# tyfeld/MMaDA-Parallel

Hardware: NVIDIA H100
Metric: denoised_tokens_per_sec (higher is better)
Workload: dtype bf16; 1 GPU; MMaDA-Parallel-A 8B, 1 prompt per GPU, 512x512 (1024 VQ tokens) + 256 text tokens, timesteps=64, text_steps=128, cfg_img=4.0, cfg_scale=0, temperature=1.0, text_temperature=0 (BASELINE configs[1]); seq_len=2414, parallelism=replicas x1 (independent prompts, no collective), weights=synthetic normal(0, 0.02) bf16, seeded, l2=16.2 GB of weights streamed per forward >> 50 MB L2 (no flush needed)

## Files before the change

### mmada_parallel_b200/csrc/attention.cu

```cuda
#include "mmdp_internal.h"
#include "ptx.cuh"

#include <stdlib.h>

#include <map>
#include <mutex>
#include <utility>

namespace mmdp {

static constexpr int kAttnThreads = 384;
static constexpr int kQBytes = 128 * 128 * 2;
template <int BKV> struct AttnCfg {
    static constexpr int kKBytes = BKV * 128 * 2;
    static constexpr int kVBytes = 128 * BKV * 2;
    static constexpr int kSmem = kQBytes + 2 * (kKBytes + kVBytes) + 1024  + 256 ;
};

__device__ __forceinline__ float ex2_approx(float x) {
    float y;
    asm("ex2.approx.ftz.f32 %0, %1;" : "=f"(y) : "f"(x));
    return y;
}

struct AttnSegs {
    int n;
    int start[kMaxSegs + 1];
    int tile0[kMaxSegs + 1];
};

template <int kBKV, bool kPacked>
__device__ __forceinline__ void attention_body(const CUtensorMap& tmQ, const CUtensorMap& tmK, const CUtensorMap& tmVt,
                                               __nv_bfloat16* __restrict__ out, int H, int L, int d_model, float scale_log2,
                                               int n_full, int splits, float* __restrict__ part_ws, int Lq, const AttnSegs* segs) {
    constexpr int kKBytes = AttnCfg<kBKV>::kKBytes, kVBytes = AttnCfg<kBKV>::kVBytes;
    extern __shared__ uint8_t smem_raw[];
    uint8_t* smem = reinterpret_cast<uint8_t*>((reinterpret_cast<uintptr_t>(smem_raw) + 1023) & ~uintptr_t(1023));
    uint8_t* sQ = smem;
    uint8_t* sK = sQ + kQBytes;
    uint8_t* sV = sK + 2 * kKBytes;
    uint64_t* bars = reinterpret_cast<uint64_t*>(sV + 2 * kVBytes);
    uint64_t* q_full = bars + 0;
    uint64_t* k_full = bars + 1;
    uint64_t* k_empty = bars + 3;
    uint64_t* v_full = bars + 5;
    uint64_t* v_empty = bars + 7;

    const int warp = threadIdx.x >> 5, lane = threadIdx.x & 31, wg = warp >> 2;
    int n_qt = (Lq + 127) / 128;
    int n_kv_all = (L + kBKV - 1) / kBKV;
    int tile = blockIdx.x, piece = -1;
    if ((int)blockIdx.x >= n_full) {
        const int t = (int)blockIdx.x - n_full;
        tile = n_full + t / splits;
        piece = t - (t / splits) * splits;
// ... 38 lines not shown
        setmaxnreg_dec<40>();
        if (warp == 0 && elect_one_sync()) {
            const int qrow0 = (kPacked ? seg0 : b * Lq) + qt * 128;
            mbar_expect_tx(q_full, kQBytes);
            tma_load_2d(sQ, &tmQ, q_full, h * 128, qrow0);
            tma_load_2d(sQ + kQBytes / 2, &tmQ, q_full, h * 128 + 64, qrow0);
            for (int j = 0; j < n_kv; ++j) {
                const int st = j & 1;
                const uint32_t ph = (j >> 1) & 1;
                const int kv0 = (jb + j) * kBKV;
                mbar_wait(&k_empty[st], ph ^ 1);
                mbar_expect_tx(&k_full[st], kKBytes);
                tma_load_2d(sK + st * kKBytes, &tmK, &k_full[st], h * 128, (kPacked ? seg0 : b * L) + kv0);
                tma_load_2d(sK + st * kKBytes + kKBytes / 2, &tmK, &k_full[st], h * 128 + 64, (kPacked ? seg0 : b * L) + kv0);
                mbar_wait(&v_empty[st], ph ^ 1);
                mbar_expect_tx(&v_full[st], kVBytes);
                tma_load_2d(sV + st * kVBytes, &tmVt, &v_full[st], kv0, (b * H + h) * 128);
                if (kBKV == 128) tma_load_2d(sV + st * kVBytes + kVBytes / 2, &tmVt, &v_full[st], kv0 + 64, (b * H + h) * 128);
            }
        }
        __syncwarp();
        return;
    }

    setmaxnreg_inc<232>();
    const int half = wg - 1;
    const int r0 = half * 64 + (warp & 3) * 16 + (lane >> 2), c0 = 2 * (lane & 3);
    const uint32_t aQ = smem_u32(sQ) + half * (64 * 128);
    float o[64];
#pragma unroll
    for (int i = 0; i < 64; ++i) o[i] = 0.f;
    float m_run[2] = {-INFINITY, -INFINITY}, l_run[2] = {0.f, 0.f};
    mbar_wait(q_full, 0);
    for (int j = 0; j < n_kv; ++j) {
        const int st = j & 1;
        const uint32_t ph = (j >> 1) & 1;
        const int nvalid = L - (jb + j) * kBKV;
        float sacc[kBKV / 2];
        const uint32_t aK = smem_u32(sK + st * kKBytes);
        mbar_wait(&k_full[st], ph);
        wgmma_fence();
#pragma unroll
        for (int kk = 0; kk < 8; ++kk)
        {
            const uint64_t qd = smem_desc_kmajor_sw128(aQ + (kk >> 2) * (kQBytes / 2)) + (kk & 3) * 2;
            const uint64_t kd = smem_desc_kmajor_sw128(aK + (kk >> 2) * (kKBytes / 2)) + (kk & 3) * 2;
            if constexpr (kBKV == 128) wgmma_bf16_ss_n128(sacc, qd, kd, kk != 0);
            else wgmma_bf16_ss_n64(sacc, qd, kd, kk != 0);
        }
        wgmma_commit();
        wgmma_wait<0>();
        reg_fence(sacc);
        __syncwarp();
        if (lane == 0) mbar_arrive(&k_empty[st]);
        if (nvalid < kBKV) {
#pragma unroll
            for (int jj = 0; jj < kBKV / 8; ++jj)
#pragma unroll
                for (int e = 0; e < 2; ++e)
                    if (8 * jj + c0 + e >= nvalid) { sacc[4 * jj + e] = -INFINITY; sacc[4 * jj + 2 + e] = -INFINITY; }
        }
        float alpha[2], mneg[2];
#pragma unroll
        for (int hh = 0; hh < 2; ++hh) {
            float mx = sacc[2 * hh];
#pragma unroll
            for (int jj = 0; jj < kBKV / 8; ++jj) mx = fmaxf(mx, fmaxf(sacc[4 * jj + 2 * hh], sacc[4 * jj + 2 * hh + 1]));
            mx = fmaxf(mx, __shfl_xor_sync(0xffffffffu, mx, 1));
            mx = fmaxf(mx, __shfl_xor_sync(0xffffffffu, mx, 2));
            const float m_new = fmaxf(m_run[hh], mx);
            alpha[hh] = ex2_approx((m_run[hh] - m_new) * scale_log2);
            m_run[hh] = m_new;
            mneg[hh] = -m_new * scale_log2;
        }
        uint32_t pa[kBKV / 4];
        float rsum[2] = {0.f, 0.f};
#pragma unroll
        for (int jj = 0; jj < kBKV / 8; ++jj)
#pragma unroll
            for (int hh = 0; hh < 2; ++hh) {
                const float p0 = ex2_approx(fmaf(sacc[4 * jj + 2 * hh], scale_log2, mneg[hh]));
                const float p1 = ex2_approx(fmaf(sacc[4 * jj + 2 * hh + 1], scale_log2, mneg[hh]));
                rsum[hh] += p0 + p1;
                pa[2 * jj + hh] = pack_bf16x2(p0, p1);
            }
#pragma unroll
        for (int hh = 0; hh < 2; ++hh) l_run[hh] = fmaf(l_run[hh], alpha[hh], rsum[hh]);
#pragma unroll
        for (int jj = 0; jj < 16; ++jj) {
            o[4 * jj] *= alpha[0]; o[4 * jj + 1] *= alpha[0];
            o[4 * jj + 2] *= alpha[1]; o[4 * jj + 3] *= alpha[1];
        }
        const uint32_t aV = smem_u32(sV + st * kVBytes);
        mbar_wait(&v_full[st], ph);
        wgmma_fence();
#pragma unroll
        for (int kk = 0; kk < kBKV / 16; ++kk) {
            const uint32_t a[4] = {pa[4 * kk], pa[4 * kk + 1], pa[4 * kk + 2], pa[4 * kk + 3]};
            wgmma_bf16_rs_n128(o, a, smem_desc_kmajor_sw128(aV + (kk >> 2) * (kVBytes / 2)) + (kk & 3) * 2, 1);
        }
        wgmma_commit();
        wgmma_wait<0>();
        reg_fence(o);
        __syncwarp();
        if (lane == 0) mbar_arrive(&v_empty[st]);
    }
#pragma unroll
    for (int hh = 0; hh < 2; ++hh) {
        l_run[hh] += __shfl_xor_sync(0xffffffffu, l_run[hh], 1);
        l_run[hh] += __shfl_xor_sync(0xffffffffu, l_run[hh], 2);
    }
#pragma unroll
    for (int hh = 0; hh < 2; ++hh) {
        const int r = r0 + 8 * hh, qrow = qt * 128 + r;
        if (qrow >= Lq) continue;
        if (piece >= 0) {
            float* slot = part_ws + (size_t)((tile - n_full) * splits + piece) * (128 * 128 + 256);
            if ((lane & 3) == 0) {
                slot[128 * 128 + r] = m_run[hh];
                slot[128 * 128 + 128 + r] = l_run[hh];
            }
#pragma unroll
            for (int jj = 0; jj < 16; ++jj)
                *reinterpret_cast<float2*>(slot + (size_t)r * 128 + 8 * jj + c0) = make_float2(o[4 * jj + 2 * hh], o[4 * jj + 2 * hh + 1]);
        } else {
            const float inv_l = 1.0f / l_run[hh];
            __nv_bfloat16* orow = out + (size_t)((kPacked ? seg0 : b * Lq) + qrow) * d_model + h * 128;
#pragma unroll
            for (int jj = 0; jj < 16; ++jj)
                *reinterpret_cast<uint32_t*>(orow + 8 * jj + c0) = pack_bf16x2(o[4 * jj + 2 * hh] * inv_l, o[4 * jj + 2 * hh + 1] * inv_l);
        }
    }
}

template <int kBKV>
__global__ void __launch_bounds__(kAttnThreads, 1)
attention_kernel(const __grid_constant__ CUtensorMap tmQ, const __grid_constant__ CUtensorMap tmK,
                 const __grid_constant__ CUtensorMap tmVt, __nv_bfloat16* __restrict__ out, int H, int L, int d_model,
                 float scale_log2, int n_full, int splits, float* __restrict__ part_ws, int Lq) {
    attention_body<kBKV, false>(tmQ, tmK, tmVt, out, H, L, d_model, scale_log2, n_full, splits, part_ws, Lq, nullptr);
}

template <int kBKV>
__global__ void __launch_bounds__(kAttnThreads, 1)
attention_packed_kernel(const __grid_constant__ CUtensorMap tmQ, const __grid_constant__ CUtensorMap tmK,
                        const __grid_constant__ CUtensorMap tmVt, __nv_bfloat16* __restrict__ out, int H, int d_model,
                        float scale_log2, int n_full, int splits, float* __restrict__ part_ws, const __grid_constant__ AttnSegs segs) {
    attention_body<kBKV, true>(tmQ, tmK, tmVt, out, H, 0, d_model, scale_log2, n_full, splits, part_ws, 0, &segs);
}

template <bool kPacked>
__device__ __forceinline__ void attention_combine_body(const float* __restrict__ part_ws, __nv_bfloat16* __restrict__ out, int H,
                                                       int Lq, int d_model, float scale_log2, int n_full, int splits,
                                                       const AttnSegs* segs) {
    int n_qt = (Lq + 127) / 128;
    const int st = blockIdx.x, r = blockIdx.y, c = threadIdx.x;
    pdl_launch_dependents();
    pdl_wait();
    const int tile = n_full + st;
    int seg = 0, seg0 = 0, tl = tile;
    if constexpr (kPacked) {
        for (int i = 1; i < segs->n; ++i)
            if (tile >= segs->tile0[i]) seg = i;
        seg0 = segs->start[seg];
        Lq = segs->start[seg + 1] - seg0;
        n_qt = (Lq + 127) / 128;
        tl = tile - segs->tile0[seg];
    }
    const int qt = tl % n_qt, h = (tl / n_qt) % H, b = kPacked ? seg : tile / (n_qt * H);
    const int qrow = qt * 128 + r;
    if (qrow >= Lq) return;
    const float* base = part_ws + (size_t)st * splits * (128 * 128 + 256);
    float m = -INFINITY;
    for (int i = 0; i < splits; ++i) m = fmaxf(m, base[(size_t)i * (128 * 128 + 256) + 128 * 128 + r]);
    float o = 0.f, l = 0.f;
    for (int i = 0; i < splits; ++i) {
        const float* slot = base + (size_t)i * (128 * 128 + 256);
        const float w = exp2f((slot[128 * 128 + r] - m) * scale_log2);
        o = fmaf(w, slot[(size_t)r * 128 + c], o);
        l = fmaf(w, slot[128 * 128 + 128 + r], l);
    }
// ... 38 lines not shown
        for (int t = first; t < tiles; ++t)
            if (sp > kvb_of(t) / 2) sp = kvb_of(t) / 2;
        auto empty_piece = [&](int s) {
            for (int t = first; t < tiles; ++t) {
                const int n_kvb = kvb_of(t);
                if ((s - 1) * ((n_kvb + s - 1) / s) >= n_kvb) return true;
            }
            return false;
        };
        while (sp >= 2 && empty_piece(sp)) --sp;
        return sp;
    };
    if (split_tail && tiles > slots && (tiles % slots) > 0 && (tiles % slots) * 4 <= slots) {
        n_split = tiles % slots;
        splits = fit_splits(slots / n_split, tiles - n_split);
        if (splits >= 2) n_full = tiles - n_split; else { n_split = 0; splits = 1; }
    } else if (split_tail && tiles * 2 <= slots) {
        splits = fit_splits(slots / tiles, 0);
        if (splits >= 2) { n_split = tiles; n_full = 0; } else splits = 1;
    }
}

template <class Kernel>
static int attn_smem_attr(Kernel kernel, int smem, unsigned long long& attr_set) {
    int dev = 0;
    MMDP_CUDA(cudaGetDevice(&dev));
    if (!(attr_set >> (dev & 63) & 1ull)) {
        MMDP_CUDA(cudaFuncSetAttribute(kernel, cudaFuncAttributeMaxDynamicSharedMemorySize, smem));
        attr_set |= 1ull << (dev & 63);
    }
    return 0;
}

template <int kBKV>
static int attention_launch(const __nv_bfloat16* q, const __nv_bfloat16* k, const __nv_bfloat16* vt, __nv_bfloat16* out, int B, int H,
                            int L, int Lpad, float scale, cudaStream_t stream, int Lq) {
    constexpr int kAttnSmem = AttnCfg<kBKV>::kSmem;
    if (B <= 0 || H <= 0 || L <= 0) return set_error("attention: empty problem");
    if (Lq <= 0) Lq = L;
    if (Lpad < L || (Lpad % 8)) return set_error("attention: Lpad must be >= L and a multiple of 8");
    const int d_model = H * 128;
    CUtensorMap tmQ, tmK, tmVt;
    if (make_tmap_2d_bf16(&tmQ, q, (uint64_t)B * Lq, (uint64_t)d_model, (uint64_t)d_model, 128, 64)) return -1;
    if (make_tmap_2d_bf16(&tmK, k, (uint64_t)B * L, (uint64_t)d_model, (uint64_t)d_model, kBKV, 64)) return -1;
    if (make_tmap_2d_bf16(&tmVt, vt, (uint64_t)B * H * 128, (uint64_t)Lpad, (uint64_t)Lpad, 128, 64)) return -1;
    const int n_qt = (Lq + 127) / 128, n_kvb = (L + kBKV - 1) / kBKV;
    const int tiles = n_qt * H * B;
    int n_full, n_split, splits;
    plan_split_tail(tiles, [&](int) { return n_kvb; }, n_full, n_split, splits);
    float* part_ws = nullptr;
    if (n_split > 0 && attn_part_workspace(stream, (size_t)n_split * splits * (128 * 128 + 256) * sizeof(float), &part_ws)) return -1;
    const int grid = n_full + n_split * splits;
    const float scale_log2 = scale * 1.4426950408889634f;
    const bool pdl = pdl_mode() != 0;
    LaunchScope ls(LK_ATTN, 4.0 * B * H * (double)Lq * L * 128, stream);
    static unsigned long long attr_set = 0;
    if (attn_smem_attr(attention_kernel<kBKV>, kAttnSmem, attr_set)) return -1;
    MMDP_CUDA(launch_ex(attention_kernel<kBKV>, dim3(grid), dim3(kAttnThreads), kAttnSmem, stream, pdl, false, tmQ, tmK, tmVt, out, H, L,
                        d_model, scale_log2, n_full, splits, part_ws, Lq));
    if (n_split > 0)
        MMDP_CUDA(launch_ex(attention_combine_kernel, dim3(n_split, 128), dim3(128), 0, stream, pdl, false, (const float*)part_ws, out, H, Lq,
                            d_model, scale_log2, n_full, splits));
    return 0;
}

template <int kBKV>
static int attention_packed_launch(const __nv_bfloat16* q, const __nv_bfloat16* k, const __nv_bfloat16* vt, __nv_bfloat16* out,
                                   const SegTable& segs, int H, int Lpad, float scale, cudaStream_t stream) {
    constexpr int kAttnSmem = AttnCfg<kBKV>::kSmem;
    if (segs.n <= 0 || segs.n > kMaxSegs || H <= 0) return set_error("attention_packed: %d sequences (1 to %d)", segs.n, kMaxSegs);
    if (Lpad % 8) return set_error("attention_packed: Lpad must be a multiple of 8");
    AttnSegs as{};
    as.n = segs.n;
    double work = 0;
    for (int s = 0; s <= segs.n; ++s) {
        as.start[s] = segs.start[s];
        if (s == segs.n) break;
        const int len = segs.start[s + 1] - segs.start[s];
        if (len <= 0 || len > Lpad) return set_error("attention_packed: sequence %d has length %d (Lpad %d)", s, len, Lpad);
        as.tile0[s + 1] = as.tile0[s] + (len + 127) / 128 * H;
        work += 4.0 * H * (double)len * len * 128;
    }
    const int M = segs.start[segs.n], tiles = as.tile0[segs.n], d_model = H * 128;
    CUtensorMap tmQ, tmK, tmVt;
    if (make_tmap_2d_bf16(&tmQ, q, (uint64_t)M, (uint64_t)d_model, (uint64_t)d_model, 128, 64)) return -1;
    if (make_tmap_2d_bf16(&tmK, k, (uint64_t)M, (uint64_t)d_model, (uint64_t)d_model, kBKV, 64)) return -1;
    if (make_tmap_2d_bf16(&tmVt, vt, (uint64_t)segs.n * H * 128, (uint64_t)Lpad, (uint64_t)Lpad, 128, 64)) return -1;
    auto kvb_of = [&](int t) {
        int s = 0;
        while (s + 1 < segs.n && t >= as.tile0[s + 1]) ++s;
        return (segs.start[s + 1] - segs.start[s] + kBKV - 1) / kBKV;
    };
    int n_full, n_split, splits;
    plan_split_tail(tiles, kvb_of, n_full, n_split, splits);
    float* part_ws = nullptr;
    if (n_split > 0 && attn_part_workspace(stream, (size_t)n_split * splits * (128 * 128 + 256) * sizeof(float), &part_ws)) return -1;
    const int grid = n_full + n_split * splits;
    const float scale_log2 = scale * 1.4426950408889634f;
    const bool pdl = pdl_mode() != 0;
    LaunchScope ls(LK_ATTN, work, stream);
    static unsigned long long attr_set = 0;
    if (attn_smem_attr(attention_packed_kernel<kBKV>, kAttnSmem, attr_set)) return -1;
    MMDP_CUDA(launch_ex(attention_packed_kernel<kBKV>, dim3(grid), dim3(kAttnThreads), kAttnSmem, stream, pdl, false, tmQ, tmK, tmVt, out,
                        H, d_model, scale_log2, n_full, splits, part_ws, as));
    if (n_split > 0)
        MMDP_CUDA(launch_ex(attention_packed_combine_kernel, dim3(n_split, 128), dim3(128), 0, stream, pdl, false, (const float*)part_ws,
                            out, H, d_model, scale_log2, n_full, splits, as));
    return 0;
}

int attention_fwd(const __nv_bfloat16* q, const __nv_bfloat16* k, const __nv_bfloat16* vt, __nv_bfloat16* out, int B, int H, int L,
                  int Lpad, float scale, cudaStream_t stream, int Lq) {
    const int version = opt(OPT_ATTN_VERSION);
    if (version == 7) return attention_launch<64>(q, k, vt, out, B, H, L, Lpad, scale, stream, Lq);
    if (version != 6) return set_error("attention: unknown kernel generation %d (6 or 7)", version);
    return attention_launch<128>(q, k, vt, out, B, H, L, Lpad, scale, stream, Lq);
}

int attention_packed_fwd(const __nv_bfloat16* q, const __nv_bfloat16* k, const __nv_bfloat16* vt, __nv_bfloat16* out,
                         const SegTable& segs, int H, int Lpad, float scale, cudaStream_t stream) {
    const int version = opt(OPT_ATTN_VERSION);
    if (version == 7) return attention_packed_launch<64>(q, k, vt, out, segs, H, Lpad, scale, stream);
    if (version != 6) return set_error("attention: unknown kernel generation %d (6 or 7)", version);
    return attention_packed_launch<128>(q, k, vt, out, segs, H, Lpad, scale, stream);
}

}
```

### mmada_parallel_b200/csrc/mmdp_internal.h

```cpp
#pragma once
#include <cuda.h>
#include <cuda_bf16.h>
#include <cuda_runtime.h>
#include <stdint.h>
#include <stdio.h>

namespace mmdp {

enum Epilogue { EPI_PLAIN = 0, EPI_RESID = 1, EPI_QKVROPE = 2, EPI_SWIGLU = 3, EPI_F32 = 4, EPI_QKVROPE_PACKED = 5 };

static constexpr int kMaxSegs = 64;
struct SegTable {
    int n;
    int start[kMaxSegs + 1];
};

int set_error(const char* fmt, ...);
const char* last_error();
int num_sms();

enum LaunchKind { LK_GEMM = 0, LK_ATTN = 1, LK_ROW = 2, LK_SAMPLE = 3, LK_COUNT = 4 };
struct LaunchScope {
    LaunchScope(int kind, double work, cudaStream_t s);
    ~LaunchScope();
    int idx;
    cudaStream_t stream;
};
void prof_enable(int on);
int prof_summary(double* ms, double* work, long long* launches);
long long launch_count(int reset);

int pdl_mode();
void set_pdl_mode(int on);
int env_int(const char* name, int dflt);
enum OptId { OPT_PDL = 0, OPT_GEMM_SPLITK, OPT_GEMM_L2PF, OPT_GEMM_L2PF_MOD, OPT_GEMM_GROUP_M, OPT_ATTN_SPLIT_TAIL,
             OPT_RMSNORM_WARP, OPT_ROW_WINDOW, OPT_ATTN_VERSION, OPT_GEMM_PAIR, OPT_COUNT };
int opt(int id);
int set_opt(const char* key, int value);

template <typename... KArgs, typename... Args>
inline cudaError_t launch_ex(void (*kernel)(KArgs...), dim3 grid, dim3 block, size_t smem, cudaStream_t stream, bool pdl,
                             bool coop, Args&&... args) {
    cudaLaunchConfig_t cfg{};
    cfg.gridDim = grid;
    cfg.blockDim = block;
    cfg.dynamicSmemBytes = smem;
    cfg.stream = stream;
    cudaLaunchAttribute at[2];
    unsigned n = 0;
    if (pdl) {
        at[n].id = cudaLaunchAttributeProgrammaticStreamSerialization;
        at[n].val.programmaticStreamSerializationAllowed = 1;
        ++n;
    }
    if (coop) {
        at[n].id = cudaLaunchAttributeCooperative;
        at[n].val.cooperative = 1;
        ++n;
    }
    cfg.attrs = at;
    cfg.numAttrs = n;
    return cudaLaunchKernelEx(&cfg, kernel, static_cast<KArgs>(args)...);
}

#define MMDP_CUDA(expr)                                                                              \
    do {                                                                                             \
        cudaError_t _e = (expr);                                                                     \
        if (_e != cudaSuccess)                                                                       \
            return ::mmdp::set_error("%s:%d: %s -> %s", __FILE__, __LINE__, #expr, cudaGetErrorString(_e)); \
// ... 97 lines not shown
```

### mmada_parallel_b200/csrc/ptx.cuh

```cuda
#pragma once
#include <cuda.h>
#include <cuda_bf16.h>
#include <cuda_runtime.h>
#include <stdint.h>

namespace mmdp {

__device__ __forceinline__ uint32_t smem_u32(const void* p) {
    return static_cast<uint32_t>(__cvta_generic_to_shared(p));
}

__device__ __forceinline__ bool elect_one_sync() {
    uint32_t pred;
    asm volatile(
        "{\n\t.reg .pred p;\n\t"
        "elect.sync _|p, 0xffffffff;\n\t"
        "selp.u32 %0, 1, 0, p;\n\t}"
        : "=r"(pred));
    return pred != 0;
}

#ifndef MMDP_WAIT_SPIN_LIMIT
#define MMDP_WAIT_SPIN_LIMIT (1u << 26)
#endif

__device__ __forceinline__ void mbar_init(uint64_t* bar, uint32_t count) {
    asm volatile("mbarrier.init.shared::cta.b64 [%0], %1;" ::"r"(smem_u32(bar)), "r"(count));
}
__device__ __forceinline__ void fence_barrier_init() {
    asm volatile("fence.mbarrier_init.release.cluster;" ::: "memory");
}
__device__ __forceinline__ void mbar_expect_tx(uint64_t* bar, uint32_t bytes) {
    asm volatile("mbarrier.arrive.expect_tx.shared::cta.b64 _, [%0], %1;" ::"r"(smem_u32(bar)), "r"(bytes)
                 : "memory");
}
__device__ __forceinline__ void mbar_arrive(uint64_t* bar) {
    asm volatile("mbarrier.arrive.shared::cta.b64 _, [%0];" ::"r"(smem_u32(bar)) : "memory");
}
__device__ __forceinline__ bool mbar_try_wait(uint64_t* bar, uint32_t parity) {
    uint32_t ok;
    asm volatile(
        "{\n\t.reg .pred p;\n\t"
        "mbarrier.try_wait.parity.shared::cta.b64 p, [%1], %2;\n\t"
        "selp.b32 %0, 1, 0, p;\n\t}"
        : "=r"(ok)
        : "r"(smem_u32(bar)), "r"(parity)
        : "memory");
    return ok != 0;
}
__device__ __forceinline__ void mbar_wait(uint64_t* bar, uint32_t parity) {
    uint32_t spins = 0;
    while (!mbar_try_wait(bar, parity)) {
        if (++spins > MMDP_WAIT_SPIN_LIMIT) __trap();
    }
}

__device__ __forceinline__ void fence_proxy_async_smem() {
    asm volatile("fence.proxy.async.shared::cta;" ::: "memory");
}

__device__ __forceinline__ void tma_prefetch_desc(const CUtensorMap* tm) {
    asm volatile("prefetch.tensormap [%0];" ::"l"(reinterpret_cast<uint64_t>(tm)) : "memory");
}
__device__ __forceinline__ void tma_load_2d(void* smem_dst, const CUtensorMap* tm, uint64_t* bar, int c0, int c1) {
    asm volatile(
        "cp.async.bulk.tensor.2d.shared::cluster.global.mbarrier::complete_tx::bytes [%0], [%1, {%3, %4}], [%2];"
        ::"r"(smem_u32(smem_dst)), "l"(reinterpret_cast<uint64_t>(tm)), "r"(smem_u32(bar)), "r"(c0), "r"(c1)
        : "memory");
}

__device__ __forceinline__ void tma_load_2d_multicast(void* smem_dst, const CUtensorMap* tm, uint64_t* bar, int c0, int c1,
                                                      uint16_t cta_mask) {
    asm volatile(
        "cp.async.bulk.tensor.2d.shared::cluster.global.mbarrier::complete_tx::bytes.multicast::cluster [%0], [%1, {%3, %4}], [%2], %5;"
        ::"r"(smem_u32(smem_dst)), "l"(reinterpret_cast<uint64_t>(tm)), "r"(smem_u32(bar)), "r"(c0), "r"(c1), "h"(cta_mask)
        : "memory");
}

__device__ __forceinline__ uint32_t cluster_ctarank() {
    uint32_t r;
    asm volatile("mov.u32 %0, %%cluster_ctarank;" : "=r"(r));
    return r;
}
__device__ __forceinline__ void cluster_sync() {
    asm volatile("barrier.cluster.arrive.release.aligned;\n\tbarrier.cluster.wait.acquire.aligned;" ::: "memory");
}
__device__ __forceinline__ void mbar_arrive_cluster(uint64_t* bar, uint32_t cta) {
// ... 134 lines not shown
```

### mmada_parallel_b200/csrc/runtime.cu

```cuda
#include "mmdp_internal.h"

#include <stdarg.h>
#include <stdlib.h>
#include <string.h>

#include <mutex>
#include <unordered_map>
#include <vector>

namespace mmdp {

static thread_local char g_err[1024] = "";

int set_error(const char* fmt, ...) {
    va_list ap;
    va_start(ap, fmt);
    vsnprintf(g_err, sizeof(g_err), fmt, ap);
    va_end(ap);
    return -1;
}
const char* last_error() { return g_err; }

int num_sms() {
    static int n = 0;
    if (n == 0) {
        int dev = 0;
        cudaDeviceProp prop;
        if (cudaGetDevice(&dev) != cudaSuccess || cudaGetDeviceProperties(&prop, dev) != cudaSuccess) return 132;
        n = prop.multiProcessorCount;
    }
    return n;
}

int env_int(const char* name, int dflt) {
    const char* e = getenv(name);
    return (e && *e) ? atoi(e) : dflt;
}

struct Opt { const char* key; const char* env; int dflt; int val; bool init; };
static Opt g_opts[OPT_COUNT] = {
    {"pdl", "MMDP_PDL", 1, 0, false},
    {"gemm_splitk", "MMDP_GEMM_SPLITK", 2, 0, false},
    {"gemm_l2pf", "MMDP_GEMM_L2PF", 0, 0, false},
    {"gemm_l2pf_mod", "MMDP_GEMM_L2PF_MOD", 4, 0, false},
    {"gemm_group_m", "MMDP_GEMM_GROUP_M", -1, 0, false},
    {"attn_split_tail", "MMDP_ATTN_SPLIT_TAIL", 1, 0, false},
    {"rmsnorm_warp", "MMDP_RMSNORM_WARP", 1, 0, false},
    {"row_window", "MMDP_ROW_WINDOW", 1, 0, false},
    {"attn_version", "MMDP_ATTN_VERSION", 6, 0, false},
    {"gemm_pair", "MMDP_GEMM_PAIR", 0, 0, false},
};
int opt(int id) {
    Opt& o = g_opts[id];
    if (!o.init) { o.val = env_int(o.env, o.dflt); o.init = true; }
    return o.val;
}
int set_opt(const char* key, int value) {
    for (int i = 0; i < OPT_COUNT; ++i)
        if (!strcmp(g_opts[i].key, key)) { g_opts[i].val = value; g_opts[i].init = true; return 0; }
    return set_error("mmdp_set_option: unknown option '%s'", key);
}
int pdl_mode() { return opt(OPT_PDL) ? 1 : 0; }
void set_pdl_mode(int on) { set_opt("pdl", on ? 1 : 0); }

struct ProfRec { cudaEvent_t e0, e1; int kind; double work; };
static std::vector<ProfRec> g_prof;
static size_t g_prof_used = 0;
static bool g_prof_on = false;
static long long g_launches = 0;

LaunchScope::LaunchScope(int kind, double work, cudaStream_t s) : idx(-1), stream(s) {
    ++g_launches;
    if (!g_prof_on) return;
    if (g_prof_used == g_prof.size()) {
        ProfRec r{};
        if (cudaEventCreate(&r.e0) != cudaSuccess || cudaEventCreate(&r.e1) != cudaSuccess) return;
        g_prof.push_back(r);
    }
    idx = (int)g_prof_used++;
    g_prof[idx].kind = kind;
    g_prof[idx].work = work;
    cudaEventRecord(g_prof[idx].e0, s);
}
// ... 108 lines not shown
```

Measured before the change: 106.1 tokens/s.

## Add persistent pipelined attention kernel overlapping QK^T with PV via ping-pong warpgroups

Adds a persistent, warp-specialized attention kernel. One producer warp streams Q/K/V tiles through a 2-stage TMA ring, and two consumer warpgroups alternate via named barriers so that each S=QK^T wgmma overlaps the previous block's PV wgmma and the other group's softmax. The grid is capped at the SM count and each CTA loops over work items, amortizing setup and Q loads. It is enabled by default through a new attn_pipeline option, at the cost of more barrier complexity and a risk of ping-pong deadlock or serialization.

After: 107.0 tokens/s, median of 6. No clear change (+0.8%).

```diff
diff --git a/mmada_parallel_b200/csrc/attention.cu b/mmada_parallel_b200/csrc/attention.cu
--- a/mmada_parallel_b200/csrc/attention.cu
+++ b/mmada_parallel_b200/csrc/attention.cu
@@ -226,20 +226,292 @@
     }
 }
 
-template <int kBKV>
+static constexpr int kPipeStages = 2;
+static constexpr int kPipeSmem = kQBytes + kPipeStages * (AttnCfg<128>::kKBytes + AttnCfg<128>::kVBytes) + 1024 + 256;
+static constexpr uint32_t kBarTurn = 1;
+
+struct AttnItem {
+    int tile, piece, qt, h, b, seg0, L, Lq, jb, n_kv;
+};
+template <bool kPacked>
+__device__ __forceinline__ AttnItem attn_item(int w, int H, int L, int Lq, int n_full, int splits, const AttnSegs* segs) {
+    AttnItem it;
+    it.tile = w; it.piece = -1;
+    if (w >= n_full) {
+        const int t = w - n_full;
+        it.tile = n_full + t / splits;
+        it.piece = t - (t / splits) * splits;
+    }
+    int seg = 0, tl = it.tile;
+    it.seg0 = 0;
+    if constexpr (kPacked) {
+        for (int i = 1; i < segs->n; ++i)
+            if (it.tile >= segs->tile0[i]) seg = i;
+        it.seg0 = segs->start[seg];
+        L = Lq = segs->start[seg + 1] - it.seg0;
+        tl = it.tile - segs->tile0[seg];
+    }
+    const int n_qt = (Lq + 127) / 128, n_kv_all = (L + 127) / 128;
+    it.qt = tl % n_qt; it.h = (tl / n_qt) % H; it.b = kPacked ? seg : it.tile / (n_qt * H);
+    it.L = L; it.Lq = Lq;
+    int jb = 0, je = n_kv_all;
+    if (it.piece >= 0) {
+        const int per = (n_kv_all + splits - 1) / splits;
+        jb = it.piece * per;
+        je = (jb + per < n_kv_all) ? jb + per : n_kv_all;
+    }
+    it.jb = jb; it.n_kv = je - jb;
+    return it;
+}
+
+__device__ __forceinline__ void attn_softmax_block(float (&sacc)[64], int nvalid, int c0, float scale_log2, float (&m_run)[2],
+                                                   float (&l_run)[2], float (&alpha)[2]) {
+    if (nvalid < 128) {
+#pragma unroll
+        for (int jj = 0; jj < 16; ++jj)
+#pragma unroll
+            for (int e = 0; e < 2; ++e)
+                if (8 * jj + c0 + e >= nvalid) { sacc[4 * jj + e] = -INFINITY; sacc[4 * jj + 2 + e] = -INFINITY; }
+    }
+    float mneg[2];
+#pragma unroll
+    for (int hh = 0; hh < 2; ++hh) {
+        float mx = sacc[2 * hh];
+#pragma unroll
+        for (int jj = 0; jj < 16; ++jj) mx = fmaxf(mx, fmaxf(sacc[4 * jj + 2 * hh], sacc[4 * jj + 2 * hh + 1]));
+        mx = fmaxf(mx, __shfl_xor_sync(0xffffffffu, mx, 1));
+        mx = fmaxf(mx, __shfl_xor_sync(0xffffffffu, mx, 2));
+        const float m_new = fmaxf(m_run[hh], mx);
+        alpha[hh] = ex2_approx((m_run[hh] - m_new) * scale_log2);
+        m_run[hh] = m_new;
+        mneg[hh] = -m_new * scale_log2;
+    }
+    float rsum[2] = {0.f, 0.f};
+#pragma unroll
+    for (int jj = 0; jj < 16; ++jj)
+#pragma unroll
+        for (int hh = 0; hh < 2; ++hh) {
+            const float p0 = ex2_approx(fmaf(sacc[4 * jj + 2 * hh], scale_log2, mneg[hh]));
+            const float p1 = ex2_approx(fmaf(sacc[4 * jj + 2 * hh + 1], scale_log2, mneg[hh]));
+            rsum[hh] += p0 + p1;
+            sacc[4 * jj + 2 * hh] = p0;
+            sacc[4 * jj + 2 * hh + 1] = p1;
+        }
+#pragma unroll
+    for (int hh = 0; hh < 2; ++hh) l_run[hh] = fmaf(l_run[hh], alpha[hh], rsum[hh]);
+}
+
+__device__ __forceinline__ void attn_pack_p(const float (&sacc)[64], uint32_t (&pa)[32]) {
+#pragma unroll
+    for (int jj = 0; jj < 16; ++jj)
+#pragma unroll
+        for (int hh = 0; hh < 2; ++hh) pa[2 * jj + hh] = pack_bf16x2(sacc[4 * jj + 2 * hh], sacc[4 * jj + 2 * hh + 1]);
+}
+
+__device__ __forceinline__ void attn_rescale_o(float (&o)[64], const float (&alpha)[2]) {
+#pragma unroll
+    for (int jj = 0; jj < 16; ++jj) {
+        o[4 * jj] *= alpha[0]; o[4 * jj + 1] *= alpha[0];
+        o[4 * jj + 2] *= alpha[1]; o[4 * jj + 3] *= alpha[1];
+    }
+}
+
+__device__ __forceinline__ void attn_issue_s(float (&sacc)[64], uint32_t aQ, uint32_t aK) {
+#pragma unroll
+    for (int kk = 0; kk < 8; ++kk) {
+        const uint64_t qd = smem_desc_kmajor_sw128(aQ + (kk >> 2) * (kQBytes / 2)) + (kk & 3) * 2;
+        const uint64_t kd = smem_desc_kmajor_sw128(aK + (kk >> 2) * (AttnCfg<128>::kKBytes / 2)) + (kk & 3) * 2;
+        wgmma_bf16_ss_n128(sacc, qd, kd, kk != 0);
+    }
+}
+
+__device__ __forceinline__ void attn_issue_pv(float (&o)[64], const uint32_t (&pa)[32], uint32_t aV) {
+#pragma unroll
+    for (int kk = 0; kk < 8; ++kk) {
+        const uint32_t a[4] = {pa[4 * kk], pa[4 * kk + 1], pa[4 * kk + 2], pa[4 * kk + 3]};
+        wgmma_bf16_rs_n128(o, a, smem_desc_kmajor_sw128(aV + (kk >> 2) * (AttnCfg<128>::kVBytes / 2)) + (kk & 3) * 2, 1);
+    }
+}
+
+template <bool kPacked>
+__device__ __forceinline__ void attention_body_pipelined(const CUtensorMap& tmQ, const CUtensorMap& tmK, const CUtensorMap& tmVt,
+                                                         __nv_bfloat16* __restrict__ out, int H, int L, int d_model,
+                                                         float scale_log2, int n_full, int splits, float* __restrict__ part_ws,
+                                                         int Lq, const AttnSegs* segs, int n_items) {
+    constexpr int kKBytes = AttnCfg<128>::kKBytes, kVBytes = AttnCfg<128>::kVBytes, S = kPipeStages;
+    extern __shared__ uint8_t smem_raw[];
+    uint8_t* smem = reinterpret_cast<uint8_t*>((reinterpret_cast<uintptr_t>(smem_raw) + 1023) & ~uintptr_t(1023));
+    uint8_t* sQ = smem;
+    uint8_t* sK = sQ + kQBytes;
+    uint8_t* sV = sK + S * kKBytes;
+    uint64_t* bars = reinterpret_cast<uint64_t*>(sV + S * kVBytes);
+    uint64_t* q_full = bars + 0;
+    uint64_t* q_empty = bars + 1;
+    uint64_t* k_full = bars + 2;
+    uint64_t* k_empty = bars + 2 + S;
+    uint64_t* v_full = bars + 2 + 2 * S;
+    uint64_t* v_empty = bars + 2 + 3 * S;
+
+    const int warp = threadIdx.x >> 5, lane = threadIdx.x & 31, wg = warp >> 2;
+    if (warp == 0 && lane == 0) {
+        tma_prefetch_desc(&tmQ);
+        tma_prefetch_desc(&tmK);
+        tma_prefetch_desc(&tmVt);
+        mbar_init(q_full, 1);
+        mbar_init(q_empty, 8);
+        for (int s = 0; s < S; ++s) {
+            mbar_init(&k_full[s], 1);
+            mbar_init(&k_empty[s], 8);
+            mbar_init(&v_full[s], 1);
+            mbar_init(&v_empty[s], 8);
+        }
+        fence_barrier_init();
+    }
+    __syncthreads();
+    pdl_launch_dependents();
+    pdl_wait();
+
+    if (wg == 0) {
+        setmaxnreg_dec<24>();
+        if (warp == 0 && elect_one_sync()) {
+            int st = 0;
+            uint32_t ph = 0, qph = 0;
+            for (int w = blockIdx.x; w < n_items; w += gridDim.x, qph ^= 1) {
+                const AttnItem it = attn_item<kPacked>(w, H, L, Lq, n_full, splits, segs);
+                const int row0 = kPacked ? it.seg0 : it.b * it.L;
+                const int qrow0 = (kPacked ? it.seg0 : it.b * it.Lq) + it.qt * 128;
+                const int vrow = (it.b * H + it.h) * 128;
+                mbar_wait(q_empty, qph ^ 1);
+                mbar_expect_tx(q_full, kQBytes);
+                tma_load_2d(sQ, &tmQ, q_full, it.h * 128, qrow0);
+                tma_load_2d(sQ + kQBytes / 2, &tmQ, q_full, it.h * 128 + 64, qrow0);
+                for (int j = 0; j < it.n_kv; ++j) {
+                    const int kv0 = (it.jb + j) * 128;
+                    mbar_wait(&k_empty[st], ph ^ 1);
+                    mbar_expect_tx(&k_full[st], kKBytes);
+                    tma_load_2d(sK + st * kKBytes, &tmK, &k_full[st], it.h * 128, row0 + kv0);
+                    tma_load_2d(sK + st * kKBytes + kKBytes / 2, &tmK, &k_full[st], it.h * 128 + 64, row0 + kv0);
+                    mbar_wait(&v_empty[st], ph ^ 1);
+                    mbar_expect_tx(&v_full[st], kVBytes);
+                    tma_load_2d(sV + st * kVBytes, &tmVt, &v_full[st], kv0, vrow);
+                    tma_load_2d(sV + st * kVBytes + kVBytes / 2, &tmVt, &v_full[st], kv0 + 64, vrow);
+                    if (++st == S) { st = 0; ph ^= 1; }
+                }
+            }
+        }
+        __syncwarp();
+        return;
+    }
+
+    setmaxnreg_inc<240>();
+    const int half = wg - 1;
+    const uint32_t bar_mine = kBarTurn + half, bar_other = kBarTurn + (half ^ 1);
+    const int r0 = half * 64 + (warp & 3) * 16 + (lane >> 2), c0 = 2 * (lane & 3);
+    const uint32_t aQ = smem_u32(sQ) + half * (64 * 128);
+    if (half == 1) named_bar_arrive(bar_other, 256);
+    int st = 0;
+    uint32_t ph = 0, qph = 0;
+    bool ok = true;
+    for (int w = blockIdx.x; w < n_items; w += gridDim.x, qph ^= 1) {
+        const AttnItem it = attn_item<kPacked>(w, H, L, Lq, n_full, splits, segs);
+        float o[64];
+#pragma unroll
+        for (int i = 0; i < 64; ++i) o[i] = 0.f;
+        float m_run[2] = {-INFINITY, -INFINITY}, l_run[2] = {0.f, 0.f}, alpha[2];
+        float sacc[64];
+        uint32_t pa[32];
+        ok &= mbar_wait_bounded(q_full, qph);
+        int pst = 0;
+        uint32_t pph = 0;
+        for (int j = 0; j < it.n_kv; ++j) {
+            ok &= mbar_wait_bounded(&k_full[st], ph);
+            if (j > 0) ok &= mbar_wait_bounded(&v_full[pst], pph);
+            named_bar_sync(bar_mine, 256);
+            wgmma_fence();
+            attn_issue_s(sacc, aQ, smem_u32(sK + st * kKBytes));
+            wgmma_commit();
+            if (j > 0) attn_issue_pv(o, pa, smem_u32(sV + pst * kVBytes));
+            wgmma_commit();
+            named_bar_arrive(bar_other, 256);
+            wgmma_wait<1>();
+            reg_fence(sacc);
+            __syncwarp();
+            if (lane == 0) {
+                mbar_arrive(&k_empty[st]);
+                if (j == it.n_kv - 1) mbar_arrive(q_empty);
+            }
+            attn_softmax_block(sacc, it.L - (it.jb + j) * 128, c0, scale_log2, m_run, l_run, alpha);
+            wgmma_wait<0>();
+            reg_fence(o);
+            __syncwarp();
+            if (j > 0 && lane == 0) mbar_arrive(&v_empty[pst]);
+            attn_rescale_o(o, alpha);
+            attn_pack_p(sacc, pa);
+            pst = st; pph = ph;
+            if (++st == S) { st = 0; ph ^= 1; }
+        }
+        ok &= mbar_wait_bounded(&v_full[pst], pph);
+        named_bar_sync(bar_mine, 256);
+        wgmma_fence();
+        attn_issue_pv(o, pa, smem_u32(sV + pst * kVBytes));
+        wgmma_commit();
+        named_bar_arrive(bar_other, 256);
+        wgmma_wait<0>();
+        reg_fence(o);
+        __syncwarp();
+        if (lane == 0) mbar_arrive(&v_empty[pst]);
+#pragma unroll
+        for (int hh = 0; hh < 2; ++hh) {
+            l_run[hh] += __shfl_xor_sync(0xffffffffu, l_run[hh], 1);
+            l_run[hh] += __shfl_xor_sync(0xffffffffu, l_run[hh], 2);
+        }
+#pragma unroll
+        for (int hh = 0; hh < 2; ++hh) {
+            const int r = r0 + 8 * hh, qrow = it.qt * 128 + r;
+            if (qrow >= it.Lq) continue;
+            if (it.piece >= 0) {
+                float* slot = part_ws + (size_t)((it.tile - n_full) * splits + it.piece) * (128 * 128 + 256);
+                if ((lane & 3) == 0) {
+                    slot[128 * 128 + r] = m_run[hh];
+                    slot[128 * 128 + 128 + r] = l_run[hh];
+                }
+#pragma unroll
+                for (int jj = 0; jj < 16; ++jj)
+                    *reinterpret_cast<float2*>(slot + (size_t)r * 128 + 8 * jj + c0) = make_float2(o[4 * jj + 2 * hh], o[4 * jj + 2 * hh + 1]);
+            } else {
+                const float inv_l = 1.0f / l_run[hh];
+                __nv_bfloat16* orow = out + (size_t)((kPacked ? it.seg0 : it.b * it.Lq) + qrow) * d_model + it.h * 128;
+#pragma unroll
+                for (int jj = 0; jj < 16; ++jj)
+                    *reinterpret_cast<uint32_t*>(orow + 8 * jj + c0) = pack_bf16x2(o[4 * jj + 2 * hh] * inv_l, o[4 * jj + 2 * hh + 1] * inv_l);
+            }
+        }
+    }
+    if (half == 0) named_bar_sync(bar_mine, 256);
+    if (!ok) __trap();
+}
+
+template <int kBKV, bool kPipelined>
 __global__ void __launch_bounds__(kAttnThreads, 1)
 attention_kernel(const __grid_constant__ CUtensorMap tmQ, const __grid_constant__ CUtensorMap tmK,
                  const __grid_constant__ CUtensorMap tmVt, __nv_bfloat16* __restrict__ out, int H, int L, int d_model,
-                 float scale_log2, int n_full, int splits, float* __restrict__ part_ws, int Lq) {
-    attention_body<kBKV, false>(tmQ, tmK, tmVt, out, H, L, d_model, scale_log2, n_full, splits, part_ws, Lq, nullptr);
-}
-
-template <int kBKV>
+                 float scale_log2, int n_full, int splits, float* __restrict__ part_ws, int Lq, int n_items) {
+    if constexpr (kPipelined)
+        attention_body_pipelined<false>(tmQ, tmK, tmVt, out, H, L, d_model, scale_log2, n_full, splits, part_ws, Lq, nullptr, n_items);
+    else
+        attention_body<kBKV, false>(tmQ, tmK, tmVt, out, H, L, d_model, scale_log2, n_full, splits, part_ws, Lq, nullptr);
+}
+
+template <int kBKV, bool kPipelined>
 __global__ void __launch_bounds__(kAttnThreads, 1)
 attention_packed_kernel(const __grid_constant__ CUtensorMap tmQ, const __grid_constant__ CUtensorMap tmK,
                         const __grid_constant__ CUtensorMap tmVt, __nv_bfloat16* __restrict__ out, int H, int d_model,
-                        float scale_log2, int n_full, int splits, float* __restrict__ part_ws, const __grid_constant__ AttnSegs segs) {
-    attention_body<kBKV, true>(tmQ, tmK, tmVt, out, H, 0, d_model, scale_log2, n_full, splits, part_ws, 0, &segs);
+                        float scale_log2, int n_full, int splits, float* __restrict__ part_ws, const __grid_constant__ AttnSegs segs,
+                        int n_items) {
+    if constexpr (kPipelined)
+        attention_body_pipelined<true>(tmQ, tmK, tmVt, out, H, 0, d_model, scale_log2, n_full, splits, part_ws, 0, &segs, n_items);
+    else
+        attention_body<kBKV, true>(tmQ, tmK, tmVt, out, H, 0, d_model, scale_log2, n_full, splits, part_ws, 0, &segs);
 }
 
 template <bool kPacked>
@@ -344,10 +616,10 @@
     return 0;
 }
 
-template <int kBKV>
+template <int kBKV, bool kPipelined>
 static int attention_launch(const __nv_bfloat16* q, const __nv_bfloat16* k, const __nv_bfloat16* vt, __nv_bfloat16* out, int B, int H,
                             int L, int Lpad, float scale, cudaStream_t stream, int Lq) {
-    constexpr int kAttnSmem = AttnCfg<kBKV>::kSmem;
+    constexpr int kAttnSmem = kPipelined ? kPipeSmem : AttnCfg<kBKV>::kSmem;
     if (B <= 0 || H <= 0 || L <= 0) return set_error("attention: empty problem");
     if (Lq <= 0) Lq = L;
     if (Lpad < L || (Lpad % 8)) return set_error("attention: Lpad must be >= L and a multiple of 8");
@@ -362,24 +634,25 @@
     plan_split_tail(tiles, [&](int) { return n_kvb; }, n_full, n_split, splits);
     float* part_ws = nullptr;
     if (n_split > 0 && attn_part_workspace(stream, (size_t)n_split * splits * (128 * 128 + 256) * sizeof(float), &part_ws)) return -1;
-    const int grid = n_full + n_split * splits;
+    const int n_items = n_full + n_split * splits;
+    const int grid = kPipelined && n_items > num_sms() ? num_sms() : n_items;
     const float scale_log2 = scale * 1.4426950408889634f;
     const bool pdl = pdl_mode() != 0;
     LaunchScope ls(LK_ATTN, 4.0 * B * H * (double)Lq * L * 128, stream);
     static unsigned long long attr_set = 0;
-    if (attn_smem_attr(attention_kernel<kBKV>, kAttnSmem, attr_set)) return -1;
-    MMDP_CUDA(launch_ex(attention_kernel<kBKV>, dim3(grid), dim3(kAttnThreads), kAttnSmem, stream, pdl, false, tmQ, tmK, tmVt, out, H, L,
-                        d_model, scale_log2, n_full, splits, part_ws, Lq));
+    if (attn_smem_attr(attention_kernel<kBKV, kPipelined>, kAttnSmem, attr_set)) return -1;
+    MMDP_CUDA(launch_ex(attention_kernel<kBKV, kPipelined>, dim3(grid), dim3(kAttnThreads), kAttnSmem, stream, pdl, false, tmQ, tmK, tmVt,
+                        out, H, L, d_model, scale_log2, n_full, splits, part_ws, Lq, n_items));
     if (n_split > 0)
         MMDP_CUDA(launch_ex(attention_combine_kernel, dim3(n_split, 128), dim3(128), 0, stream, pdl, false, (const float*)part_ws, out, H, Lq,
                             d_model, scale_log2, n_full, splits));
     return 0;
 }
 
-template <int kBKV>
+template <int kBKV, bool kPipelined>
 static int attention_packed_launch(const __nv_bfloat16* q, const __nv_bfloat16* k, const __nv_bfloat16* vt, __nv_bfloat16* out,
                                    const SegTable& segs, int H, int Lpad, float scale, cudaStream_t stream) {
-    constexpr int kAttnSmem = AttnCfg<kBKV>::kSmem;
+    constexpr int kAttnSmem = kPipelined ? kPipeSmem : AttnCfg<kBKV>::kSmem;
     if (segs.n <= 0 || segs.n > kMaxSegs || H <= 0) return set_error("attention_packed: %d sequences (1 to %d)", segs.n, kMaxSegs);
     if (Lpad % 8) return set_error("attention_packed: Lpad must be a multiple of 8");
     AttnSegs as{};
@@ -407,14 +680,15 @@
     plan_split_tail(tiles, kvb_of, n_full, n_split, splits);
     float* part_ws = nullptr;
     if (n_split > 0 && attn_part_workspace(stream, (size_t)n_split * splits * (128 * 128 + 256) * sizeof(float), &part_ws)) return -1;
-    const int grid = n_full + n_split * splits;
+    const int n_items = n_full + n_split * splits;
+    const int grid = kPipelined && n_items > num_sms() ? num_sms() : n_items;
     const float scale_log2 = scale * 1.4426950408889634f;
     const bool pdl = pdl_mode() != 0;
     LaunchScope ls(LK_ATTN, work, stream);
     static unsigned long long attr_set = 0;
-    if (attn_smem_attr(attention_packed_kernel<kBKV>, kAttnSmem, attr_set)) return -1;
-    MMDP_CUDA(launch_ex(attention_packed_kernel<kBKV>, dim3(grid), dim3(kAttnThreads), kAttnSmem, stream, pdl, false, tmQ, tmK, tmVt, out,
-                        H, d_model, scale_log2, n_full, splits, part_ws, as));
+    if (attn_smem_attr(attention_packed_kernel<kBKV, kPipelined>, kAttnSmem, attr_set)) return -1;
+    MMDP_CUDA(launch_ex(attention_packed_kernel<kBKV, kPipelined>, dim3(grid), dim3(kAttnThreads), kAttnSmem, stream, pdl, false, tmQ, tmK,
+                        tmVt, out, H, d_model, scale_log2, n_full, splits, part_ws, as, n_items));
     if (n_split > 0)
         MMDP_CUDA(launch_ex(attention_packed_combine_kernel, dim3(n_split, 128), dim3(128), 0, stream, pdl, false, (const float*)part_ws,
                             out, H, d_model, scale_log2, n_full, splits, as));
@@ -424,17 +698,19 @@
 int attention_fwd(const __nv_bfloat16* q, const __nv_bfloat16* k, const __nv_bfloat16* vt, __nv_bfloat16* out, int B, int H, int L,
                   int Lpad, float scale, cudaStream_t stream, int Lq) {
     const int version = opt(OPT_ATTN_VERSION);
-    if (version == 7) return attention_launch<64>(q, k, vt, out, B, H, L, Lpad, scale, stream, Lq);
+    if (version == 7) return attention_launch<64, false>(q, k, vt, out, B, H, L, Lpad, scale, stream, Lq);
     if (version != 6) return set_error("attention: unknown kernel generation %d (6 or 7)", version);
-    return attention_launch<128>(q, k, vt, out, B, H, L, Lpad, scale, stream, Lq);
+    if (opt(OPT_ATTN_PIPELINE)) return attention_launch<128, true>(q, k, vt, out, B, H, L, Lpad, scale, stream, Lq);
+    return attention_launch<128, false>(q, k, vt, out, B, H, L, Lpad, scale, stream, Lq);
 }
 
 int attention_packed_fwd(const __nv_bfloat16* q, const __nv_bfloat16* k, const __nv_bfloat16* vt, __nv_bfloat16* out,
                          const SegTable& segs, int H, int Lpad, float scale, cudaStream_t stream) {
     const int version = opt(OPT_ATTN_VERSION);
-    if (version == 7) return attention_packed_launch<64>(q, k, vt, out, segs, H, Lpad, scale, stream);
+    if (version == 7) return attention_packed_launch<64, false>(q, k, vt, out, segs, H, Lpad, scale, stream);
     if (version != 6) return set_error("attention: unknown kernel generation %d (6 or 7)", version);
-    return attention_packed_launch<128>(q, k, vt, out, segs, H, Lpad, scale, stream);
-}
-
-}
+    if (opt(OPT_ATTN_PIPELINE)) return attention_packed_launch<128, true>(q, k, vt, out, segs, H, Lpad, scale, stream);
+    return attention_packed_launch<128, false>(q, k, vt, out, segs, H, Lpad, scale, stream);
+}
+
+}
diff --git a/mmada_parallel_b200/csrc/mmdp_internal.h b/mmada_parallel_b200/csrc/mmdp_internal.h
--- a/mmada_parallel_b200/csrc/mmdp_internal.h
+++ b/mmada_parallel_b200/csrc/mmdp_internal.h
@@ -34,7 +34,8 @@
 void set_pdl_mode(int on);
 int env_int(const char* name, int dflt);
 enum OptId { OPT_PDL = 0, OPT_GEMM_SPLITK, OPT_GEMM_L2PF, OPT_GEMM_L2PF_MOD, OPT_GEMM_GROUP_M, OPT_ATTN_SPLIT_TAIL,
-             OPT_RMSNORM_WARP, OPT_ROW_WINDOW, OPT_ATTN_VERSION, OPT_GEMM_PAIR, OPT_COUNT };
+             OPT_RMSNORM_WARP, OPT_ROW_WINDOW, OPT_ATTN_VERSION, OPT_GEMM_PAIR,
+             OPT_ATTN_PIPELINE, OPT_COUNT };
 int opt(int id);
 int set_opt(const char* key, int value);
 
diff --git a/mmada_parallel_b200/csrc/ptx.cuh b/mmada_parallel_b200/csrc/ptx.cuh
--- a/mmada_parallel_b200/csrc/ptx.cuh
+++ b/mmada_parallel_b200/csrc/ptx.cuh
@@ -53,6 +53,21 @@
     while (!mbar_try_wait(bar, parity)) {
         if (++spins > MMDP_WAIT_SPIN_LIMIT) __trap();
     }
+}
+
+__device__ __forceinline__ void named_bar_sync(uint32_t id, uint32_t threads) {
+    asm volatile("bar.sync %0, %1;" ::"r"(id), "r"(threads) : "memory");
+}
+__device__ __forceinline__ void named_bar_arrive(uint32_t id, uint32_t threads) {
+    asm volatile("bar.arrive %0, %1;" ::"r"(id), "r"(threads) : "memory");
+}
+
+__device__ __forceinline__ bool mbar_wait_bounded(uint64_t* bar, uint32_t parity) {
+    uint32_t spins = 0;
+    while (!mbar_try_wait(bar, parity)) {
+        if (++spins > MMDP_WAIT_SPIN_LIMIT) return false;
+    }
+    return true;
 }
 
 __device__ __forceinline__ void fence_proxy_async_smem() {
diff --git a/mmada_parallel_b200/csrc/runtime.cu b/mmada_parallel_b200/csrc/runtime.cu
--- a/mmada_parallel_b200/csrc/runtime.cu
+++ b/mmada_parallel_b200/csrc/runtime.cu
@@ -49,6 +49,7 @@
     {"row_window", "MMDP_ROW_WINDOW", 1, 0, false},
     {"attn_version", "MMDP_ATTN_VERSION", 6, 0, false},
     {"gemm_pair", "MMDP_GEMM_PAIR", 0, 0, false},
+    {"attn_pipeline", "MMDP_ATTN_PIPELINE", 1, 0, false},
 };
 int opt(int id) {
     Opt& o = g_opts[id];
```

## Software-pipeline attention: overlap PV of block j-1 with QK of block j, ping-pong warpgroups

Applied to the files above, without the earlier changes.

Restructures the attention consumer loop so the P·V wgmma for the previous KV block is issued together with the Q·K wgmma for the current block, and the softmax of one block overlaps with tensor-core work. Two named barriers alternate the two consumer warpgroups so one issues wgmma while the other does softmax, in the FlashAttention-3 ping-pong style. The intent is to hide softmax/exp latency behind tensor-core execution. It adds a bounded-spin wait with a trap on timeout, keeps more live registers (pa plus sacc plus o), and complicates the barrier protocol.

After: 105.9 tokens/s before, 106.6 tokens/s after (median of 6 runs). About the same (+0.7%).

```diff
diff --git a/mmada_parallel_b200/csrc/attention.cu b/mmada_parallel_b200/csrc/attention.cu
--- a/mmada_parallel_b200/csrc/attention.cu
+++ b/mmada_parallel_b200/csrc/attention.cu
@@ -21,6 +21,94 @@
     float y;
     asm("ex2.approx.ftz.f32 %0, %1;" : "=f"(y) : "f"(x));
     return y;
+}
+
+template <int kBKV>
+__device__ __forceinline__ void attn_issue_qk(float (&sacc)[kBKV / 2], uint32_t aQ, uint32_t aK) {
+#pragma unroll
+    for (int kk = 0; kk < 8; ++kk) {
+        const uint64_t qd = smem_desc_kmajor_sw128(aQ + (kk >> 2) * (kQBytes / 2)) + (kk & 3) * 2;
+        const uint64_t kd = smem_desc_kmajor_sw128(aK + (kk >> 2) * (AttnCfg<kBKV>::kKBytes / 2)) + (kk & 3) * 2;
+        if constexpr (kBKV == 128) wgmma_bf16_ss_n128(sacc, qd, kd, kk != 0);
+        else wgmma_bf16_ss_n64(sacc, qd, kd, kk != 0);
+    }
+}
+
+template <int kBKV>
+__device__ __forceinline__ void attn_issue_pv(float (&o)[64], const uint32_t (&pa)[kBKV / 4], uint32_t aV) {
+#pragma unroll
+    for (int kk = 0; kk < kBKV / 16; ++kk) {
+        const uint32_t a[4] = {pa[4 * kk], pa[4 * kk + 1], pa[4 * kk + 2], pa[4 * kk + 3]};
+        wgmma_bf16_rs_n128(o, a, smem_desc_kmajor_sw128(aV + (kk >> 2) * (AttnCfg<kBKV>::kVBytes / 2)) + (kk & 3) * 2, 1);
+    }
+}
+
+template <int kBKV>
+__device__ __forceinline__ void attn_softmax_block(float (&sacc)[kBKV / 2], int nvalid, int c0, float scale_log2, float (&m_run)[2],
+                                                   float (&l_run)[2], float (&alpha)[2]) {
+    if (nvalid < kBKV) {
+#pragma unroll
+        for (int jj = 0; jj < kBKV / 8; ++jj)
+#pragma unroll
+            for (int e = 0; e < 2; ++e)
+                if (8 * jj + c0 + e >= nvalid) { sacc[4 * jj + e] = -INFINITY; sacc[4 * jj + 2 + e] = -INFINITY; }
+    }
+    float mneg[2];
+#pragma unroll
+    for (int hh = 0; hh < 2; ++hh) {
+        float mx = sacc[2 * hh];
+#pragma unroll
+        for (int jj = 0; jj < kBKV / 8; ++jj) mx = fmaxf(mx, fmaxf(sacc[4 * jj + 2 * hh], sacc[4 * jj + 2 * hh + 1]));
+        mx = fmaxf(mx, __shfl_xor_sync(0xffffffffu, mx, 1));
+        mx = fmaxf(mx, __shfl_xor_sync(0xffffffffu, mx, 2));
+        const float m_new = fmaxf(m_run[hh], mx);
+        alpha[hh] = ex2_approx((m_run[hh] - m_new) * scale_log2);
+        m_run[hh] = m_new;
+        mneg[hh] = -m_new * scale_log2;
+    }
+    float rsum[2] = {0.f, 0.f};
+#pragma unroll
+    for (int jj = 0; jj < kBKV / 8; ++jj)
+#pragma unroll
+        for (int hh = 0; hh < 2; ++hh) {
+            const float p0 = ex2_approx(fmaf(sacc[4 * jj + 2 * hh], scale_log2, mneg[hh]));
+            const float p1 = ex2_approx(fmaf(sacc[4 * jj + 2 * hh + 1], scale_log2, mneg[hh]));
+            rsum[hh] += p0 + p1;
+            sacc[4 * jj + 2 * hh] = p0;
+            sacc[4 * jj + 2 * hh + 1] = p1;
+        }
+#pragma unroll
+    for (int hh = 0; hh < 2; ++hh) l_run[hh] = fmaf(l_run[hh], alpha[hh], rsum[hh]);
+}
+
+template <int kBKV>
+__device__ __forceinline__ void attn_pack_p(const float (&p)[kBKV / 2], uint32_t (&pa)[kBKV / 4]) {
+#pragma unroll
+    for (int jj = 0; jj < kBKV / 8; ++jj)
+#pragma unroll
+        for (int hh = 0; hh < 2; ++hh) pa[2 * jj + hh] = pack_bf16x2(p[4 * jj + 2 * hh], p[4 * jj + 2 * hh + 1]);
+}
+
+__device__ __forceinline__ void attn_rescale_o(float (&o)[64], const float (&alpha)[2]) {
+#pragma unroll
+    for (int jj = 0; jj < 16; ++jj) {
+        o[4 * jj] *= alpha[0]; o[4 * jj + 1] *= alpha[0];
+        o[4 * jj + 2] *= alpha[1]; o[4 * jj + 3] *= alpha[1];
+    }
+}
+
+__device__ __forceinline__ uint32_t attn_wait(uint64_t* bar, uint32_t parity) {
+    uint32_t spins = 0;
+    while (!mbar_try_wait(bar, parity))
+        if (++spins > MMDP_WAIT_SPIN_LIMIT) return 1;
+    return 0;
+}
+
+__device__ __forceinline__ void named_bar_sync(uint32_t id, uint32_t count) {
+    asm volatile("bar.sync %0, %1;" ::"r"(id), "r"(count) : "memory");
+}
+__device__ __forceinline__ void named_bar_arrive(uint32_t id, uint32_t count) {
+    asm volatile("bar.arrive %0, %1;" ::"r"(id), "r"(count) : "memory");
 }
 
 struct AttnSegs {
@@ -125,78 +213,66 @@
     for (int i = 0; i < 64; ++i) o[i] = 0.f;
     float m_run[2] = {-INFINITY, -INFINITY}, l_run[2] = {0.f, 0.f};
     mbar_wait(q_full, 0);
-    for (int j = 0; j < n_kv; ++j) {
-        const int st = j & 1;
-        const uint32_t ph = (j >> 1) & 1;
-        const int nvalid = L - (jb + j) * kBKV;
-        float sacc[kBKV / 2];
-        const uint32_t aK = smem_u32(sK + st * kKBytes);
-        mbar_wait(&k_full[st], ph);
-        wgmma_fence();
-#pragma unroll
-        for (int kk = 0; kk < 8; ++kk)
+    {
+        const uint32_t my_bar = 1 + half, other_bar = 2 - half;
+        if (half == 1) named_bar_arrive(other_bar, 256);
+        uint32_t pa[kBKV / 4];
+        uint32_t lost = 0;
+        auto softmax = [&](int j, float (&sacc)[kBKV / 2]) {
+            float alpha[2];
+            attn_softmax_block<kBKV>(sacc, L - (jb + j) * kBKV, c0, scale_log2, m_run, l_run, alpha);
+            attn_pack_p<kBKV>(sacc, pa);
+            attn_rescale_o(o, alpha);
+        };
         {
-            const uint64_t qd = smem_desc_kmajor_sw128(aQ + (kk >> 2) * (kQBytes / 2)) + (kk & 3) * 2;
-            const uint64_t kd = smem_desc_kmajor_sw128(aK + (kk >> 2) * (kKBytes / 2)) + (kk & 3) * 2;
-            if constexpr (kBKV == 128) wgmma_bf16_ss_n128(sacc, qd, kd, kk != 0);
-            else wgmma_bf16_ss_n64(sacc, qd, kd, kk != 0);
-        }
-        wgmma_commit();
-        wgmma_wait<0>();
-        reg_fence(sacc);
-        __syncwarp();
-        if (lane == 0) mbar_arrive(&k_empty[st]);
-        if (nvalid < kBKV) {
-#pragma unroll
-            for (int jj = 0; jj < kBKV / 8; ++jj)
-#pragma unroll
-                for (int e = 0; e < 2; ++e)
-                    if (8 * jj + c0 + e >= nvalid) { sacc[4 * jj + e] = -INFINITY; sacc[4 * jj + 2 + e] = -INFINITY; }
-        }
-        float alpha[2], mneg[2];
-#pragma unroll
-        for (int hh = 0; hh < 2; ++hh) {
-            float mx = sacc[2 * hh];
-#pragma unroll
-            for (int jj = 0; jj < kBKV / 8; ++jj) mx = fmaxf(mx, fmaxf(sacc[4 * jj + 2 * hh], sacc[4 * jj + 2 * hh + 1]));
-            mx = fmaxf(mx, __shfl_xor_sync(0xffffffffu, mx, 1));
-            mx = fmaxf(mx, __shfl_xor_sync(0xffffffffu, mx, 2));
-            const float m_new = fmaxf(m_run[hh], mx);
-            alpha[hh] = ex2_approx((m_run[hh] - m_new) * scale_log2);
-            m_run[hh] = m_new;
-            mneg[hh] = -m_new * scale_log2;
-        }
-        uint32_t pa[kBKV / 4];
-        float rsum[2] = {0.f, 0.f};
-#pragma unroll
-        for (int jj = 0; jj < kBKV / 8; ++jj)
-#pragma unroll
-            for (int hh = 0; hh < 2; ++hh) {
-                const float p0 = ex2_approx(fmaf(sacc[4 * jj + 2 * hh], scale_log2, mneg[hh]));
-                const float p1 = ex2_approx(fmaf(sacc[4 * jj + 2 * hh + 1], scale_log2, mneg[hh]));
-                rsum[hh] += p0 + p1;
-                pa[2 * jj + hh] = pack_bf16x2(p0, p1);
+            float sacc[kBKV / 2];
+            lost |= attn_wait(&k_full[0], 0);
+            named_bar_sync(my_bar, 256);
+            wgmma_fence();
+            attn_issue_qk<kBKV>(sacc, aQ, smem_u32(sK));
+            wgmma_commit();
+            named_bar_arrive(other_bar, 256);
+            wgmma_wait<0>();
+            reg_fence(sacc);
+            __syncwarp();
+            if (lane == 0) mbar_arrive(&k_empty[0]);
+            softmax(0, sacc);
+        }
+        for (int j = 1; j < n_kv; ++j) {
+            const int st = j & 1, pst = st ^ 1;
+            float sacc[kBKV / 2];
+            lost |= attn_wait(&k_full[st], (j >> 1) & 1);
+            lost |= attn_wait(&v_full[pst], ((j - 1) >> 1) & 1);
+            named_bar_sync(my_bar, 256);
+            wgmma_fence();
+            attn_issue_pv<kBKV>(o, pa, smem_u32(sV + pst * kVBytes));
+            attn_issue_qk<kBKV>(sacc, aQ, smem_u32(sK + st * kKBytes));
+            wgmma_commit();
+            named_bar_arrive(other_bar, 256);
+            wgmma_wait<0>();
+            reg_fence(o);
+            reg_fence(sacc);
+            __syncwarp();
+            if (lane == 0) {
+                mbar_arrive(&v_empty[pst]);
+                mbar_arrive(&k_empty[st]);
             }
-#pragma unroll
-        for (int hh = 0; hh < 2; ++hh) l_run[hh] = fmaf(l_run[hh], alpha[hh], rsum[hh]);
-#pragma unroll
-        for (int jj = 0; jj < 16; ++jj) {
-            o[4 * jj] *= alpha[0]; o[4 * jj + 1] *= alpha[0];
-            o[4 * jj + 2] *= alpha[1]; o[4 * jj + 3] *= alpha[1];
-        }
-        const uint32_t aV = smem_u32(sV + st * kVBytes);
-        mbar_wait(&v_full[st], ph);
-        wgmma_fence();
-#pragma unroll
-        for (int kk = 0; kk < kBKV / 16; ++kk) {
-            const uint32_t a[4] = {pa[4 * kk], pa[4 * kk + 1], pa[4 * kk + 2], pa[4 * kk + 3]};
-            wgmma_bf16_rs_n128(o, a, smem_desc_kmajor_sw128(aV + (kk >> 2) * (kVBytes / 2)) + (kk & 3) * 2, 1);
-        }
-        wgmma_commit();
-        wgmma_wait<0>();
-        reg_fence(o);
-        __syncwarp();
-        if (lane == 0) mbar_arrive(&v_empty[st]);
+            softmax(j, sacc);
+        }
+        {
+            const int st = (n_kv - 1) & 1;
+            lost |= attn_wait(&v_full[st], ((n_kv - 1) >> 1) & 1);
+            if (lost) __trap();
+            named_bar_sync(my_bar, 256);
+            wgmma_fence();
+            attn_issue_pv<kBKV>(o, pa, smem_u32(sV + st * kVBytes));
+            wgmma_commit();
+            if (half == 0) named_bar_arrive(other_bar, 256);
+            wgmma_wait<0>();
+            reg_fence(o);
+            __syncwarp();
+            if (lane == 0) mbar_arrive(&v_empty[st]);
+        }
     }
 #pragma unroll
     for (int hh = 0; hh < 2; ++hh) {
```
